# cbrl/BNN-PYNQ

Measured on AMD Instinct MI355X. Metric: images/sec (whole node) CNV-W1A1 CIFAR-10-shape batch, higher is better.
Workload: dtype u1; 1 GPU; cnvW1A1, 131072 synthetic 32x32x3 uint8 images per GPU per step, inputs resident in HBM, params cifar10/cnvW1A1; parallelism=dp1 (batch shards, no data-path collective)

## Files before the change

### bnn-pynq_amd/csrc/kernels.hip

```cpp
#include <hip/hip_runtime.h>
#include <hip/hip_ext.h>
#include <stdint.h>

#include <cstdlib>
#include <cstring>
#include <type_traits>

#define BNN_HD __host__ __device__
#include "act_faults.h"
#include "input_faults.h"
#include "kernels.h"
#include "mem_faults.h"
#include "mem_org.h"
#include "packed_params.h"
static_assert(bnn::kL0TileOffset == (int)bnn::kL0MfmaTileOffset && bnn::kL0BigBytes == (int)bnn::kL0MfmaBigBytes,
              "k_conv0_tile's operand offsets must be the ones packed_params.cpp writes the layer-0 table by");

namespace bnn {
namespace {

typedef const uint32_t __attribute__((address_space(4))) *kptr32;
typedef const uint64_t __attribute__((address_space(4))) *kptr64;

constexpr int kBlock = 256;
constexpr int kLfcFusedMaxA2 = 2048;

struct BlockMap { int cg, item; bool valid; };
__device__ __forceinline__ BlockMap map_block(int groups, int n_items) {
  const int bid = blockIdx.x, xcd = bid & 7, slot = bid >> 3;
  const int sg = slot / groups;
  BlockMap m;
  m.cg = slot - sg * groups;
  m.item = (sg * 8 + xcd) * kBlock + threadIdx.x;
  m.valid = m.item < n_items;
  return m;
}

struct MultiArgs {
  const MultiSeg *segs;
  unsigned stride_dw;
  int ipi;
  int res_images;
};
__device__ __forceinline__ MultiSeg multi_seg(const MultiArgs &ma) {
  kptr32 p = (kptr32)(uintptr_t)(ma.segs + blockIdx.y);
  return MultiSeg{(int)p[0], (int)p[1], (int)p[2], (int)p[3]};
}
template <typename T>
__device__ __forceinline__ int multi_prologue(const MultiArgs &ma, const uint32_t *__restrict__ &rows, T *__restrict__ &out, int &n_items, int out_per_item) {
  const MultiSeg sg = multi_seg(ma);
  rows += (size_t)sg.run * ma.stride_dw;
  n_items = sg.len * ma.ipi;
  if (ma.res_images > 0) out += ((size_t)sg.run * ma.res_images + sg.image - sg.slot) * out_per_item;
  return sg.slot * ma.ipi;
}

__device__ __forceinline__ int pc64(uint64_t x) { return __builtin_popcountll(x); }

__device__ __forceinline__ void mark_done(unsigned *done, unsigned seq, int lane) {
  if (!done) return;
  __threadfence_system();
  if (lane == 0) *reinterpret_cast<volatile unsigned *>(done) = seq;
}

template <bool OUT2, int NPB = 32>
__device__ __forceinline__ void store_bits(uint32_t *__restrict__ out, size_t pix, int groups, int g,
                                           uint32_t b0, uint32_t b1) {
  constexpr int PER64 = 64 / NPB;
  if constexpr (!OUT2) {
    if constexpr (NPB == 32) out[pix * groups + g] = b0;
    else reinterpret_cast<uint8_t *>(out)[pix * groups + g] = (uint8_t)b0;
  } else {
    const size_t w64 = pix * (groups / PER64) + g / PER64;
    const int sub = g % PER64;
    if constexpr (NPB == 32) {
      out[(w64 * 2 + 0) * 2 + sub] = b0;
      out[(w64 * 2 + 1) * 2 + sub] = b1;
    } else {
      uint8_t *o8 = reinterpret_cast<uint8_t *>(out);
      o8[(w64 * 2 + 0) * 8 + sub] = (uint8_t)b0;
      o8[(w64 * 2 + 1) * 8 + sub] = (uint8_t)b1;
    }
  }
}

template <int ARITH>
__device__ __forceinline__ void mac(int &m, int &z, uint64_t as, uint64_t az, kptr64 w) {
  if constexpr (ARITH == AR_XNOR) {
    m += pc64(w[0] ^ as);
  } else if constexpr (ARITH == AR_TB) {
    m += pc64(az & (as ^ w[0]));
  } else {
    const uint64_t zz = az & w[1];
    z += pc64(zz);
    m += pc64(zz & (as ^ w[0]));
  }
}

template <int ARITH>
constexpr int planes_in() { return ARITH == AR_XNOR ? 1 : 2; }
template <int ARITH>
constexpr int wplanes() { return ARITH == AR_TT ? 2 : 1; }
template <int ARITH, int KW>
constexpr int row_dw() { return ARITH == AR_TT ? 4 + 6 * KW : 2 + 2 * KW * wplanes<ARITH>(); }
__device__ __forceinline__ int two_extra(uint32_t two, uint32_t as, uint32_t az) {
  const uint32_t x = two & az;
  return 2 * __builtin_popcount(x & as) - __builtin_popcount(x);
}
__device__ __forceinline__ int two_extra64(uint64_t two, uint64_t as, uint64_t az) {
  const uint64_t x = two & az;
  return 2 * __builtin_popcountll(x & as) - __builtin_popcountll(x);
}

template <int ARITH>
__device__ __forceinline__ int finish(int m, int z, int nzt) {
  if constexpr (ARITH == AR_XNOR) return m;
  else if constexpr (ARITH == AR_TB) return nzt - 2 * m;
  else return z - 2 * m;
}

__device__ __forceinline__ uint32_t quantise4(uint32_t p) {
  const uint32_t t = p ^ 0x80808080u;
  const uint32_t s = (t & 0x7F7F7F7Fu) + 0x01010101u;
  const uint32_t inc = p & ~s & 0x80808080u;
  return t + (inc >> 7);
}

__device__ __forceinline__ uint32_t shift_in_sign(uint32_t bits, int v) {
  asm("" : "+v"(v));
  return __builtin_amdgcn_alignbit(bits, (uint32_t)v, 31);
}

__device__ __forceinline__ void gather_taps(const uint8_t *__restrict__ imgs, int item, uint32_t (&a)[7]) {
  const int img = item / 900, p = item - img * 900;
  const int oy = p / 30, ox = p - oy * 30;
  const uint32_t *__restrict__ im32 = reinterpret_cast<const uint32_t *>(imgs + (size_t)img * 3072);
  const uint32_t *__restrict__ row0 = im32 + oy * 8 + (ox >> 2);
  const int last = 767 - (oy * 8 + (ox >> 2));
  const int sh = ox & 3;
  uint32_t g[9];
#pragma unroll
  for (int c = 0; c < 3; c++)
#pragma unroll
    for (int r = 0; r < 3; r++) {
      const int off = c * 256 + r * 8;
      const uint32_t d0 = row0[off];
      const uint32_t d1 = (c == 2 && r == 2) ? row0[off + 1 <= last ? off + 1 : last] : row0[off + 1];
      g[c * 3 + r] = __builtin_amdgcn_alignbyte(d1, d0, sh);
    }
#pragma unroll
  for (int h = 0; h < 2; h++) {
    a[3 * h + 0] = __builtin_amdgcn_perm(g[4 * h + 1], g[4 * h + 0], 0x04020100u);
    a[3 * h + 1] = __builtin_amdgcn_perm(g[4 * h + 2], g[4 * h + 1], 0x05040201u);
    a[3 * h + 2] = __builtin_amdgcn_perm(g[4 * h + 3], g[4 * h + 2], 0x06050402u);
  }
  a[6] = g[8];
#pragma unroll
  for (int j = 0; j < 7; j++) a[j] = quantise4(a[j]);
}

template <bool OUT2, bool MULTI = false>
__global__ __launch_bounds__(kBlock) void k_conv0(const uint8_t *__restrict__ imgs, uint32_t *__restrict__ out,
                                                   const uint32_t *__restrict__ rows, int n_items, int groups, int gpb, MultiArgs ma = {}) {
  if constexpr (MULTI) {
    const MultiSeg sg = multi_seg(ma);
    rows += (size_t)sg.run * ma.stride_dw;
    n_items = sg.len * 900;
    imgs += (size_t)sg.image * 3072;
    out += (size_t)sg.slot * 900 * (OUT2 ? 4 : 2);
  }
  const BlockMap bm = map_block(groups / gpb, n_items);
  if (!bm.valid) return;
  const int item = bm.item;
  uint32_t a[7];
  gather_taps(imgs, item, a);
  for (int cg = bm.cg * gpb, cg_end = cg + gpb; cg < cg_end; cg++) {
    kptr32 w = (kptr32)(uintptr_t)(rows + (size_t)cg * 32 * 12);
    uint32_t b0 = 0, b1 = 0;
    for (int c = 31; c >= 0; c -= 2) {
      kptr32 rA = w + c * 12, rB = rA - 12;
      int accA = ~(int)rA[0], accB = ~(int)rB[0];
  #pragma unroll
      for (int k = 0; k < 7; k++) {
        accA = __builtin_amdgcn_sdot4((int)a[k], (int)rA[2 + k], accA, false);
        asm("" : "+v"(accA));
        accB = __builtin_amdgcn_sdot4((int)a[k], (int)rB[2 + k], accB, false);
        asm("" : "+v"(accB));
      }
      if constexpr (!OUT2) {
        b0 = shift_in_sign(b0, accA);
        b0 = shift_in_sign(b0, accB);
      } else {
        const int dA = accA + ((int)rA[0] - (int)rA[1]), dB = accB + ((int)rB[0] - (int)rB[1]);
        b0 = shift_in_sign(b0, accA & dA);
        b1 = shift_in_sign(b1, accA ^ dA);
        b0 = shift_in_sign(b0, accB & dB);
        b1 = shift_in_sign(b1, accB ^ dB);
      }
    }
    if constexpr (!OUT2) b0 = ~b0;
    else b1 = ~b1;
    store_bits<OUT2>(out, (size_t)item, 2, cg, b0, b1);
  }
}

typedef int v4i __attribute__((ext_vector_type(4)));
typedef int v16i __attribute__((ext_vector_type(16)));

__device__ __forceinline__ uint32_t sign_nibbles(const int (&v)[16], int h) {
  uint32_t x = 0;
#pragma unroll
  for (int g = 3; g >= 0; g--) {
#pragma unroll
    for (int q = 3; q >= 0; q--) x = shift_in_sign(x, v[4 * g + q]);
    if (g) x <<= 4;
  }
  return x << (4 * h);
}
__device__ __forceinline__ uint32_t or_halves(uint32_t x) {
  const auto sw = __builtin_amdgcn_permlane32_swap(x, x, false, false);
  return sw[0] | sw[1];
}

template <bool OUT2>
__global__ __launch_bounds__(kBlock, 2) void k_conv0_mfma(const uint8_t *__restrict__ imgs, uint32_t *__restrict__ out,
                                                        const uint8_t *__restrict__ l0tab, int n_items) {
  const int lane = threadIdx.x & 63, r = lane & 31, h = lane >> 5;
  const int pix = blockIdx.x * kBlock + threadIdx.x;
  if (pix - lane >= n_items) return;
  uint32_t t[7];
  gather_taps(imgs, pix < n_items ? pix : n_items - 1, t);
  uint32_t lo[4] = {t[0], t[1], t[2], t[3]};
  uint32_t hi[4] = {t[4], t[5], (t[6] & 0x00FFFFFFu) | 0x01000000u, 0x00000040u};
  v4i bp[2];
#pragma unroll
  for (int k = 0; k < 4; k++) {
    const auto sw = __builtin_amdgcn_permlane32_swap(lo[k], hi[k], false, false);
    bp[0][k] = (int)sw[0];
    bp[1][k] = (int)sw[1];
  }
  const v4i *__restrict__ atab = reinterpret_cast<const v4i *>(l0tab);
  uint32_t w0[2] = {0, 0}, w1[2] = {0, 0};
  const v16i zero = {0, 0, 0, 0, 0, 0, 0, 0, 0, 0, 0, 0, 0, 0, 0, 0};
#pragma unroll
  for (int ct = 0; ct < 2; ct++) {
    const v4i a = atab[(32 * ct + r) * 2 + h];
    v4i a2 = a;
    if constexpr (OUT2) a2 = atab[(64 + 32 * ct + r) * 2 + h];
#pragma unroll
    for (int pt = 0; pt < 2; pt++) {
      const v16i acc = __builtin_amdgcn_mfma_i32_32x32x32_i8(a, bp[pt], zero, 0, 0, 0);
      int v[16];
#pragma unroll
      for (int i = 0; i < 16; i++) v[i] = acc[i];
      uint32_t y0, y1 = 0;
      if constexpr (!OUT2) {
        y0 = ~or_halves(sign_nibbles(v, h));
      } else {
        const v16i acc2 = __builtin_amdgcn_mfma_i32_32x32x32_i8(a2, bp[pt], zero, 0, 0, 0);
        int u[16];
#pragma unroll
        for (int i = 0; i < 16; i++) u[i] = acc2[i];
        const uint32_t n0 = sign_nibbles(v, h), n1 = sign_nibbles(u, h);
        y0 = or_halves(n0 & n1);
        y1 = ~or_halves(n0 ^ n1);
      }
      const uint32_t mine = (pt == h) ? 0xFFFFFFFFu : 0u;
      w0[ct] |= y0 & mine;
      w1[ct] |= y1 & mine;
    }
  }
  if (pix < n_items) {
    if constexpr (!OUT2) {
      *reinterpret_cast<uint2 *>(out + (size_t)pix * 2) = make_uint2(w0[0], w0[1]);
    } else {
      *reinterpret_cast<uint4 *>(out + (size_t)pix * 4) = make_uint4(w0[0], w0[1], w1[0], w1[1]);
    }
  }
}

constexpr int kL0Imgs = 8;
constexpr int kL0Plane = 1024 + 64, kL0Image = 3 * kL0Plane;

__device__ __forceinline__ uint32_t sign_bits16(const v16i &acc) {
  uint32_t x = 0;
#pragma unroll
  for (int i = 15; i >= 0; i--) x = shift_in_sign(x, acc[i]);
  return x;
}
__device__ __forceinline__ uint32_t merge_halves(uint32_t a, uint32_t b) {
  const auto sw = __builtin_amdgcn_permlane32_swap(a, b, false, false);
  return sw[0] | sw[1];
}
template <int OFF>
__device__ __forceinline__ uint32_t lds_run(const uint32_t *aligned, uint32_t shift) {
  return __builtin_amdgcn_alignbyte(aligned[OFF / 4 + 1], aligned[OFF / 4], shift);
}

template <bool OUT2, bool MULTI = false>
__global__ __launch_bounds__(kBlock, 2) void k_conv0_tile(const uint8_t *__restrict__ imgs, uint32_t *__restrict__ out,
                                                        const uint8_t *__restrict__ l0tab, int n_images, MultiArgs ma = {}) {
  __shared__ uint4 q4[kL0Imgs * kL0Image / 16];
  const int tid = threadIdx.x, lane = tid & 63, r = lane & 31, h = lane >> 5;
  const int wave = __builtin_amdgcn_readfirstlane(tid >> 6);
  const int img0 = blockIdx.x * kL0Imgs;
  if constexpr (MULTI) {
    const MultiSeg sg = multi_seg(ma);
    if (img0 >= sg.len) return;
    l0tab += (size_t)sg.run * ma.stride_dw * 4;
    n_images = sg.len;
    imgs += (size_t)sg.image * 3072;
    out += (size_t)sg.slot * 900 * (OUT2 ? 4 : 2);
  }
  const int cnt = __builtin_amdgcn_readfirstlane(min(kL0Imgs, n_images - img0));
  const uint4 *__restrict__ src = reinterpret_cast<const uint4 *>(imgs + (size_t)img0 * 3072);
  for (int i = tid; i < cnt * 192; i += kBlock) {
    uint4 v = src[i];
    v.x = quantise4(v.x); v.y = quantise4(v.y); v.z = quantise4(v.z); v.w = quantise4(v.w);
    const int g = i / 192, j = i - g * 192;
    q4[(g * kL0Image + (j >> 6) * kL0Plane + (j & 63) * 16) >> 4] = v;
  }
  const uint8_t *__restrict__ tab = l0tab + kL0TileOffset;
  v4i abig[2];
  long asm0[2], asm1[2];
#pragma unroll
  for (int ct = 0; ct < 2; ct++) {
    abig[ct] = *reinterpret_cast<const v4i *>(tab + ((ct * 32 + r) * 2 + h) * 16);
    asm0[ct] = *reinterpret_cast<const long *>(tab + kL0BigBytes + (((0 * 2 + ct) * 32 + r) * 2 + h) * 8);
    asm1[ct] = OUT2 ? *reinterpret_cast<const long *>(tab + kL0BigBytes + (((1 * 2 + ct) * 32 + r) * 2 + h) * 8) : 0;
  }
  __syncthreads();
  const uint8_t *qb = reinterpret_cast<const uint8_t *>(q4);
  const v16i zero = {0, 0, 0, 0, 0, 0, 0, 0, 0, 0, 0, 0, 0, 0, 0, 0};
  const uint32_t lane_byte = (uint32_t)(r + h * kL0Plane);
  const bool live = r < 30;
  for (int T = wave; T < cnt * 30; T += kBlock / 64) {
    const int gi = T / 30, oy = T - gi * 30;
    const size_t pix = (size_t)(img0 + gi) * 900 + (size_t)(oy * 30) + r;
    const uint32_t byte = (uint32_t)(gi * kL0Image + 32 * oy) + lane_byte;
    const uint32_t *al = reinterpret_cast<const uint32_t *>(qb + (byte & ~3u));
    const uint32_t *al2 = reinterpret_cast<const uint32_t *>(qb + ((byte & ~3u) - h * (kL0Plane - 64)));
    v4i bb;
    bb[0] = (int)lds_run<0>(al, byte);
    bb[1] = (int)lds_run<32>(al, byte);
    bb[2] = (int)lds_run<64>(al, byte);
    bb[3] = (int)lds_run<2 * kL0Plane>(al2, byte);
    const uint32_t mid = lds_run<2 * kL0Plane + 32>(al2, byte);
    const long bs = (long)(uint64_t)(h ? 0x00004001u : mid);
    uint32_t x[2], y[2];
    v16i big[2], d0[2], d1[2];
#pragma unroll
    for (int ct = 0; ct < 2; ct++) big[ct] = __builtin_amdgcn_mfma_i32_32x32x32_i8(abig[ct], bb, zero, 0, 0, 0);
#pragma unroll
    for (int ct = 0; ct < 2; ct++) {
      d0[ct] = __builtin_amdgcn_mfma_i32_32x32x16_i8(asm0[ct], bs, big[ct], 0, 0, 0);
      if constexpr (OUT2) d1[ct] = __builtin_amdgcn_mfma_i32_32x32x16_i8(asm1[ct], bs, big[ct], 0, 0, 0);
    }
#pragma unroll
    for (int ct = 0; ct < 2; ct++) {
      if constexpr (!OUT2) {
        x[ct] = sign_bits16(d0[ct]) << (16 * h);
      } else {
        const uint32_t n0 = sign_bits16(d0[ct]), n1 = sign_bits16(d1[ct]);
        x[ct] = (n0 & n1) << (16 * h);
        y[ct] = (n0 ^ n1) << (16 * h);
      }
    }
    if constexpr (!OUT2) {
      const uint32_t w = ~merge_halves(x[0], x[1]);
      if (live) out[pix * 2 + h] = w;
    } else {
      const uint32_t sg = merge_halves(x[0], x[1]), nz = ~merge_halves(y[0], y[1]);
      if (live) {
        out[pix * 4 + h] = sg;
        out[pix * 4 + 2 + h] = nz;
      }
    }
  }
}

__global__ __launch_bounds__(kBlock) void k_l1_literal(const uint64_t *__restrict__ in, uint64_t *__restrict__ out,
                                                        const uint32_t *__restrict__ rows, int n_items) {
  __shared__ uint64_t w[64][9];
  __shared__ int thr[64];
  for (int i = threadIdx.x; i < 64 * 20; i += kBlock) {
    const int n = i / 20, j = i - n * 20;
    const uint32_t v = rows[i];
    if (j == 0) thr[n] = (int)v;
    else if (j >= 2) reinterpret_cast<uint32_t *>(&w[n][0])[j - 2] = v;
  }
  __syncthreads();
  const int item = blockIdx.x * kBlock + threadIdx.x;
  const int it = item < n_items ? item : n_items - 1;
  const int quad = it >> 2, sub = it & 3, img = quad / 196, q = quad - img * 196, qy = q / 14, qx = q - qy * 14;
  const int oy = 2 * qy + (sub >> 1), ox = 2 * qx + (sub & 1);
  const uint64_t *__restrict__ base = in + (size_t)img * 900 + (size_t)oy * 30 + ox;
  uint64_t a[9];
#pragma unroll
  for (int ky = 0; ky < 3; ky++)
#pragma unroll
    for (int kx = 0; kx < 3; kx++) a[ky * 3 + kx] = base[ky * 30 + kx];
  uint64_t bits = 0;
  for (int n = 0; n < 64; n++) {
    int m = 0;
#pragma unroll
    for (int j = 0; j < 9; j++) m += __popcll(w[n][j] ^ a[j]);
    bits |= (uint64_t)(m < thr[n]) << n;
  }
  bits |= __shfl_xor(bits, 1, 64);
  bits |= __shfl_xor(bits, 2, 64);
  if (sub == 0 && item < n_items) out[quad] = bits;
}

typedef int v8i __attribute__((ext_vector_type(8)));
typedef float v16f __attribute__((ext_vector_type(16)));
constexpr int kL1Pix = 912;

__device__ __forceinline__ uint32_t fp4_pm1(uint32_t byte) {
  uint32_t t = ~byte & 0xFFu;
  t = (t | (t << 12)) & 0x000F000Fu;
  t = (t | (t << 6)) & 0x03030303u;
  t = (t | (t << 3)) & 0x11111111u;
  return (t << 3) + 0x22222222u;
}

__global__ __launch_bounds__(256, 2) void k_l1_mfma(const uint32_t *__restrict__ in, uint32_t *__restrict__ out,
                                                     const uint8_t *__restrict__ tab, int n_images) {
  __shared__ uint4 plane[2][2][kL1Pix];
  __shared__ uint32_t lut[256];
  const int tid = threadIdx.x, lane = tid & 63, wave = tid >> 6, c = lane & 31, h = lane >> 5;
  lut[tid] = fp4_pm1((uint32_t)tid);
  const uint4 *__restrict__ wt = reinterpret_cast<const uint4 *>(tab);
  v8i wreg[9][2];
#pragma unroll
  for (int tap = 0; tap < 9; tap++)
#pragma unroll
    for (int mt = 0; mt < 2; mt++) {
      const uint4 v = wt[(tap * 2 + mt) * 64 + lane];
      wreg[tap][mt] = v8i{(int)v.x, (int)v.y, (int)v.z, (int)v.w, 0, 0, 0, 0};
    }
  __shared__ v16f seed_lds[2][2];
  if (tid < 64) reinterpret_cast<float *>(seed_lds)[tid] = reinterpret_cast<const float *>(tab + kL1MfmaWeights)[tid];
  const int cc = c < 28 ? c : 27;
  uint32_t pre[15];
  auto fetch = [&](int pair) {
    const int img0 = pair * 2, lim = min(2, n_images - img0) * 1800;
#pragma unroll
    for (int j = 0; j < 15; j++) {
      const int d = tid + 256 * j;
      pre[j] = d < lim ? in[(size_t)img0 * 1800 + d] : 0u;
    }
  };
  if (blockIdx.x * 2 < n_images) fetch(blockIdx.x);
  for (int pair = blockIdx.x; pair * 2 < n_images; pair += gridDim.x) {
    const int img0 = pair * 2, nimg = min(2, n_images - img0);
    __syncthreads();
#pragma unroll
    for (int j = 0; j < 15; j++) {
      const int d = tid + 256 * j;
      if (d < nimg * 1800) {
        const int i = d >= 1800, e = d - i * 1800, pix = e >> 1, hh = e & 1;
        const uint32_t bits = pre[j];
        plane[i][hh][pix] = make_uint4(lut[bits & 255], lut[(bits >> 8) & 255], lut[(bits >> 16) & 255], lut[bits >> 24]);
      }
    }
    if ((pair + gridDim.x) * 2 < n_images) fetch(pair + gridDim.x);
    __syncthreads();
    for (int rp = wave; rp < nimg * 14; rp += 4) {
      const int i = rp / 14, r = rp - i * 14;
      const uint4 *__restrict__ P = &plane[i][h][0];
      v16f acc[2][2] = {{seed_lds[0][h], seed_lds[0][h]}, {seed_lds[1][h], seed_lds[1][h]}};
#pragma unroll
      for (int kx = 0; kx < 3; kx++) {
        v8i b[4];
#pragma unroll
        for (int y = 0; y < 4; y++) {
          const uint4 v = P[(2 * r + y) * 30 + cc + kx];
          b[y] = v8i{(int)v.x, (int)v.y, (int)v.z, (int)v.w, 0, 0, 0, 0};
        }
#pragma unroll
        for (int ky = 0; ky < 3; ky++)
#pragma unroll
          for (int mt = 0; mt < 2; mt++)
#pragma unroll
            for (int pt = 0; pt < 2; pt++)
              acc[mt][pt] = __builtin_amdgcn_mfma_scale_f32_32x32x64_f8f6f4(wreg[ky * 3 + kx][mt], b[ky + pt], acc[mt][pt], 4, 4, 0,
                                                                              0x7F7F7F7F, 0, 0x7F7F7F7F);
      }
      uint32_t word[2];
#pragma unroll
      for (int mt = 0; mt < 2; mt++) {
        int v[16];
#pragma unroll
        for (int k = 0; k < 16; k++) v[k] = __float_as_int(fmaxf(acc[mt][0][k], acc[mt][1][k]));
        const uint32_t nf = or_halves(sign_nibbles(v, h));
        const uint32_t pooled = nf & (uint32_t)__builtin_amdgcn_mov_dpp((int)nf, 0xB1, 0xF, 0xF, true);
        word[mt] = ~pooled;
      }
      if (h == 0 && c < 28 && !(c & 1))
        *reinterpret_cast<uint2 *>(out + ((size_t)(img0 + i) * 196 + r * 14 + (c >> 1)) * 2) = make_uint2(word[0], word[1]);
    }
  }
}

constexpr int conv_mfma_row_stride(int win) {
  int ws = win;
  while ((2 * ws - (win - 2)) % 16) ws++;
  return ws;
}
constexpr int conv_mfma_img_stride(int win, int cd) {
  const int ws = conv_mfma_row_stride(win);
  int s = cd * win * ws;
  while ((s - 2 * ((win - 2) / 2 - 1) * ws - (win - 2)) % 16) s++;
  return s;
}

template <int WIN, int CD, int NT, bool POOL, int G>
__global__ __launch_bounds__(256, 2) void k_conv_mfma(const uint32_t *__restrict__ in, uint32_t *__restrict__ out,
                                                       const uint8_t *__restrict__ tab, int n_images) {
  constexpr int WOUT = WIN - 2, RP = WOUT / 2, IPI = RP * WOUT, KH = CD / 2, KS = 9 * KH, NS = 3 * KH, STREAMS = 4 / NT;
  constexpr int PIX = WIN * WIN, DWI = PIX * CD, NPF = (G * DWI + 255) / 256;
  constexpr int WS = conv_mfma_row_stride(WIN), PIXS = WIN * WS, IMGS = conv_mfma_img_stride(WIN, CD);
  static_assert(WOUT % 2 == 0 && IPI % 2 == 0 && (NT == 2 || NT == 4), "tile geometry");
  __shared__ uint4 plane[G * IMGS];
  __shared__ uint32_t lut[256];
  const int tid = threadIdx.x, lane = tid & 63, wave = __builtin_amdgcn_readfirstlane(tid >> 6), mt = wave % NT, c = lane & 31, h = lane >> 5;
  lut[tid] = fp4_pm1((uint32_t)tid);
  const uint4 *__restrict__ wt = reinterpret_cast<const uint4 *>(tab);
  v8i wreg[KS];
#pragma unroll
  for (int ks = 0; ks < KS; ks++) {
    const uint4 v = wt[(ks * NT + mt) * 64 + lane];
    wreg[ks] = v8i{(int)v.x, (int)v.y, (int)v.z, (int)v.w, 0, 0, 0, 0};
  }
  const v16f seed = reinterpret_cast<const v16f *>(tab + (size_t)KS * NT * 64 * 16)[mt * 2 + h];
  const int ngroups = (n_images + G - 1) / G;
  uint32_t pre[NPF];
  auto fetch = [&](int grp) {
    const int img0 = grp * G, lim = min(G, n_images - img0) * DWI;
#pragma unroll
    for (int j = 0; j < NPF; j++) {
      const int d = tid + 256 * j;
      pre[j] = d < lim ? in[(size_t)img0 * DWI + d] : 0u;
    }
  };
  auto slot = [&](int d) {
    const int i = d / DWI, e = d - i * DWI, pix = e / CD, q = e % CD;
    return i * IMGS + q * PIXS + (WS == WIN ? pix : pix / WIN * WS + pix % WIN);
  };
  constexpr int STEP = 32 * STREAMS, DR = STEP / WOUT, DX = STEP % WOUT, PS_LAST = (G - 1) * IMGS + 2 * (RP - 1) * WS + WOUT - 1;
  constexpr bool RAGGED = (G * IPI) % 32 != 0;
  static_assert(DX % 2 == 0 && DR + 1 <= RP, "a lane's column keeps its parity; one row-pair wrap and one image wrap per step");
  const int item0 = (wave / NT) * 32 + c, i0 = item0 / IPI, rem0 = item0 - i0 * IPI, rp0 = rem0 / WOUT, x0 = rem0 - rp0 * WOUT;
  const int ps0 = i0 * IMGS + 2 * rp0 * WS + x0;
  const uint32_t ob0 = (uint32_t)((i0 * (WOUT * WOUT) + (2 * rp0 + h) * WOUT + x0) * NT + mt) * 4;
  if (blockIdx.x < ngroups) fetch(blockIdx.x);
  for (int grp = blockIdx.x; grp < ngroups; grp += gridDim.x) {
    const int img0 = grp * G, nimg = min(G, n_images - img0), nitems = nimg * IPI;
    uint32_t *__restrict__ gout = out + (size_t)img0 * (POOL ? RP * RP : WOUT * WOUT) * NT;
    __syncthreads();
#pragma unroll
    for (int j = 0; j < NPF; j++) {
      const int d = tid + 256 * j;
      if (d < nimg * DWI) {
        const uint32_t bits = pre[j];
        plane[slot(d)] = make_uint4(lut[bits & 255], lut[(bits >> 8) & 255], lut[(bits >> 16) & 255], lut[bits >> 24]);
      }
    }
    if (grp + (int)gridDim.x < ngroups) fetch(grp + gridDim.x);
    __syncthreads();
    int x = x0, rp = rp0, ps = ps0;
    [[maybe_unused]] uint32_t ob = ob0;
    for (int t0 = (wave / NT) * 32; t0 < nitems; t0 += STEP) {
      v16f acc[2] = {seed, seed};
      const uint4 *__restrict__ P = &plane[(RAGGED ? min(ps, PS_LAST) : ps) + h * PIXS];
      auto read = [&](v8i &b, int s, int y) {
        const uint4 v = P[(s / 3) * 2 * PIXS + y * WS + s % 3];
        b = v8i{(int)v.x, (int)v.y, (int)v.z, (int)v.w, 0, 0, 0, 0};
      };
      auto mfma = [&](const v8i (&b)[4], int s, int k) {
        acc[k & 1] = __builtin_amdgcn_mfma_scale_f32_32x32x64_f8f6f4(wreg[((k >> 1) * 3 + s % 3) * KH + s / 3], b[(k >> 1) + (k & 1)], acc[k & 1], 4,
                                                                    4, 0, 0x7F7F7F7F, 0, 0x7F7F7F7F);
      };
      v8i b[2][4];
#pragma unroll
      for (int y = 0; y < 4; y++) read(b[0][y], 0, y);
#pragma unroll
      for (int s = 0; s < NS; s++)
#pragma unroll
        for (int k = 0; k < 6; k++) {
          __builtin_amdgcn_sched_barrier(0);
          mfma(b[s & 1], s, k);
          if (s + 1 < NS && k < 4) read(b[(s + 1) & 1][k], s + 1, k);
        }
      __builtin_amdgcn_sched_barrier(0);
      const bool valid = t0 + c < nitems;
      if constexpr (POOL) {
        int v[16];
#pragma unroll
        for (int k = 0; k < 16; k++) v[k] = __float_as_int(acc[0][k]) & __float_as_int(acc[1][k]);
        const uint32_t nf = or_halves(sign_nibbles(v, h));
        const uint32_t pooled = nf & (uint32_t)__builtin_amdgcn_mov_dpp((int)nf, 0xB1, 0xF, 0xF, true);
        if (valid && h == 0 && !(c & 1)) gout[(size_t)(t0 >> 1) * NT + (c >> 1) * NT + mt] = ~pooled;
      } else {
        uint32_t nf[2];
#pragma unroll
        for (int dy = 0; dy < 2; dy++) {
          int v[16];
#pragma unroll
          for (int k = 0; k < 16; k++) v[k] = __float_as_int(acc[dy][k]);
          nf[dy] = sign_nibbles(v, h);
        }
        const auto sw = __builtin_amdgcn_permlane32_swap(nf[0], nf[1], false, false);
        if (valid) *reinterpret_cast<uint32_t *>(reinterpret_cast<char *>(gout) + ob) = ~(sw[0] | sw[1]);
      }
      x += DX, rp += DR, ps += 2 * DR * WS + DX;
      if constexpr (!POOL) ob += (2 * DR * WOUT + DX) * NT * 4;
      if (x >= WOUT) {
        x -= WOUT, rp += 1, ps += 2 * WS - WOUT;
        if constexpr (!POOL) ob += WOUT * NT * 4;
      }
      if (rp >= RP) rp -= RP, ps += IMGS - 2 * RP * WS;
    }
  }
}

__global__ __launch_bounds__(256) void k_conv_mfma_table(const uint32_t *__restrict__ rows, int row_dw, int ksteps, int tiles,
                                                          int mw, uint8_t *__restrict__ dst) {
  const int idx = blockIdx.x * 256 + threadIdx.x, nw = ksteps * tiles * 64;
  if (idx < nw) {
    const int ks = idx / (tiles * 64), mt = (idx / 64) % tiles, lane = idx & 63, n = 32 * mt + (lane & 31), h = lane >> 5;
    const uint32_t bits = rows[(size_t)n * row_dw + 2 + 2 * ks + h];
    reinterpret_cast<uint4 *>(dst)[idx] = make_uint4(fp4_pm1(bits & 255), fp4_pm1((bits >> 8) & 255), fp4_pm1((bits >> 16) & 255),
                                                     fp4_pm1(bits >> 24));
  } else if (idx < nw + tiles * 32) {
    const int j = idx - nw, mt = j >> 5, h = (j >> 4) & 1, reg = j & 15;
    const int n = 32 * mt + (reg & 3) + 8 * (reg >> 2) + 4 * h;
    long long t = (int)rows[(size_t)n * row_dw];
    t = t < -1 ? -1 : (t > mw + 2 ? mw + 2 : t);
    reinterpret_cast<float *>(dst + (size_t)nw * 16)[j] = (float)(-(mw - 2 * t) - 1);
  }
}

__device__ __forceinline__ uint32_t nibble_spread(uint32_t byte) {
  uint32_t t = byte & 0xFFu;
  t = (t | (t << 12)) & 0x000F000Fu;
  t = (t | (t << 6)) & 0x03030303u;
  return (t | (t << 3)) & 0x11111111u;
}
__device__ __forceinline__ uint4 fp4_planes(const uint32_t *lutz, const uint32_t *luts, uint32_t sg, uint32_t nz) {
  const uint32_t m = sg & nz;
  return make_uint4(lutz[nz & 255] | luts[m & 255], lutz[(nz >> 8) & 255] | luts[(m >> 8) & 255],
                    lutz[(nz >> 16) & 255] | luts[(m >> 16) & 255], lutz[nz >> 24] | luts[m >> 24]);
}
__device__ __forceinline__ void not_fired(const v16f &acc, const v16f &dt, int h, uint32_t &n0, uint32_t &n1) {
  int v[16], u[16];
#pragma unroll
  for (int k = 0; k < 16; k++) {
    v[k] = __float_as_int(acc[k]);
    u[k] = __float_as_int(acc[k] - dt[k]);
  }
  n0 = or_halves(sign_nibbles(v, h));
  n1 = or_halves(sign_nibbles(u, h));
}

template <int WIN, int CD, int NT, bool POOL, int G>
__global__ __launch_bounds__(256, 2) void k_conv_mfma_a2(const uint4 *__restrict__ in, uint32_t *__restrict__ out,
                                                          const uint8_t *__restrict__ tab, int n_images) {
  constexpr int WOUT = WIN - 2, RP = WOUT / 2, IPI = RP * WOUT, KH = CD / 2, KS = 9 * KH, STREAMS = 4 / NT;
  constexpr int PIX = WIN * WIN, QWI = PIX * KH, NPF = (G * QWI + 255) / 256;
  static_assert(WOUT % 2 == 0 && IPI % 2 == 0 && (NT == 2 || NT == 4), "tile geometry");
  __shared__ uint4 plane[G][CD][PIX];
  __shared__ uint32_t lutz[256], luts[256];
  const int tid = threadIdx.x, lane = tid & 63, wave = tid >> 6, mt = wave % NT, c = lane & 31, h = lane >> 5;
  lutz[tid] = nibble_spread((uint32_t)tid) << 1;
  luts[tid] = nibble_spread((uint32_t)tid) << 3;
  const uint4 *__restrict__ wt = reinterpret_cast<const uint4 *>(tab);
  v8i wreg[KS];
#pragma unroll
  for (int ks = 0; ks < KS; ks++) {
    const uint4 v = wt[(ks * NT + mt) * 64 + lane];
    wreg[ks] = v8i{(int)v.x, (int)v.y, (int)v.z, (int)v.w, 0, 0, 0, 0};
  }
  const v16f *__restrict__ cst = reinterpret_cast<const v16f *>(tab + (size_t)KS * NT * 64 * 16);
  const v16f seed = cst[mt * 2 + h], dt = cst[NT * 2 + mt * 2 + h];
  const int ngroups = (n_images + G - 1) / G;
  uint4 pre[NPF];
  auto fetch = [&](int grp) {
    const int img0 = grp * G, lim = min(G, n_images - img0) * QWI;
#pragma unroll
    for (int j = 0; j < NPF; j++) {
      const int d = tid + 256 * j;
      pre[j] = d < lim ? in[(size_t)img0 * QWI + d] : make_uint4(0u, 0u, 0u, 0u);
    }
  };
  if (blockIdx.x < ngroups) fetch(blockIdx.x);
  for (int grp = blockIdx.x; grp < ngroups; grp += gridDim.x) {
    const int img0 = grp * G, nimg = min(G, n_images - img0), nitems = nimg * IPI;
    __syncthreads();
#pragma unroll
    for (int j = 0; j < NPF; j++) {
      const int d = tid + 256 * j;
      if (d < nimg * QWI) {
        const int i = d / QWI, e = d - i * QWI, pix = e / KH, cw = e % KH;
        const uint4 v = pre[j];
        plane[i][2 * cw][pix] = fp4_planes(lutz, luts, v.x, v.z);
        plane[i][2 * cw + 1][pix] = fp4_planes(lutz, luts, v.y, v.w);
      }
    }
    if (grp + (int)gridDim.x < ngroups) fetch(grp + gridDim.x);
    __syncthreads();
    for (int t0 = (wave / NT) * 32; t0 < nitems; t0 += 32 * STREAMS) {
      const int item = min(t0 + c, nitems - 1);
      const int i = item / IPI, rem = item - i * IPI, rp = rem / WOUT, x = rem - rp * WOUT;
      v16f acc[2] = {seed, seed};
#pragma unroll
      for (int kh = 0; kh < KH; kh++) {
        const uint4 *__restrict__ P = &plane[i][kh * 2 + h][2 * rp * WIN + x];
#pragma unroll
        for (int kx = 0; kx < 3; kx++) {
          v8i b[4];
#pragma unroll
          for (int y = 0; y < 4; y++) {
            const uint4 v = P[y * WIN + kx];
            b[y] = v8i{(int)v.x, (int)v.y, (int)v.z, (int)v.w, 0, 0, 0, 0};
          }
#pragma unroll
          for (int ky = 0; ky < 3; ky++)
#pragma unroll
            for (int dy = 0; dy < 2; dy++)
              acc[dy] = __builtin_amdgcn_mfma_scale_f32_32x32x64_f8f6f4(wreg[(ky * 3 + kx) * KH + kh], b[ky + dy], acc[dy], 4, 4, 0,
                                                                         0x7F7F7F7F, 0, 0x7F7F7F7F);
        }
      }
      const bool valid = t0 + c < nitems;
      const size_t img = (size_t)(img0 + i);
      if constexpr (POOL) {
        v16f top;
#pragma unroll
        for (int k = 0; k < 16; k++) top[k] = fmaxf(acc[0][k], acc[1][k]);
        uint32_t n0, n1;
        not_fired(top, dt, h, n0, n1);
        n0 &= (uint32_t)__builtin_amdgcn_mov_dpp((int)n0, 0xB1, 0xF, 0xF, true);
        n1 &= (uint32_t)__builtin_amdgcn_mov_dpp((int)n1, 0xB1, 0xF, 0xF, true);
        const size_t w64 = (img * (RP * RP) + rp * RP + (x >> 1)) * (NT / 2) + mt / 2;
        if (valid && !(x & 1)) out[(w64 * 2 + h) * 2 + (mt & 1)] = h ? ~(n0 ^ n1) : (n0 & n1);
      } else {
        uint32_t n0[2], n1[2];
#pragma unroll
        for (int dy = 0; dy < 2; dy++) not_fired(acc[dy], dt, h, n0[dy], n1[dy]);
        const uint32_t m0 = h ? n0[1] : n0[0], m1 = h ? n1[1] : n1[0];
        const size_t w64 = (img * (WOUT * WOUT) + (2 * rp + h) * WOUT + x) * (NT / 2) + mt / 2;
        if (valid) {
          out[(w64 * 2 + 0) * 2 + (mt & 1)] = m0 & m1;
          out[(w64 * 2 + 1) * 2 + (mt & 1)] = ~(m0 ^ m1);
        }
      }
    }
  }
}

template <bool TT>
__global__ __launch_bounds__(256) void k_conv_mfma_a2_table(const uint32_t *__restrict__ rows, int ksteps, int tiles,
                                                             uint8_t *__restrict__ dst) {
  const int idx = blockIdx.x * 256 + threadIdx.x, nw = ksteps * tiles * 64, row_dw = TT ? 4 + 6 * ksteps : 2 + 2 * ksteps;
  if (idx < nw) {
    const int ks = idx / (tiles * 64), mt = (idx / 64) % tiles, lane = idx & 63, n = 32 * mt + (lane & 31), h = lane >> 5;
    const uint32_t *__restrict__ row = rows + (size_t)n * row_dw;
    uint32_t b1, b2 = 0, b3;
    if constexpr (TT) {
      const uint32_t sg = row[2 + 4 * ks + h], two = row[2 + 4 * ksteps + 2 * ks + h], nz = row[2 + 4 * ks + 2 + h] | two;
      b1 = nz & ~two;
      b2 = two;
      b3 = (sg & nz) | two;
    } else {
      b1 = 0xFFFFFFFFu;
      b3 = row[2 + 2 * ks + h];
    }
    uint32_t v[4];
#pragma unroll
    for (int k = 0; k < 4; k++)
      v[k] = (nibble_spread(b1 >> (8 * k)) << 1) | (nibble_spread(b2 >> (8 * k)) << 2) | (nibble_spread(b3 >> (8 * k)) << 3);
    reinterpret_cast<uint4 *>(dst)[idx] = make_uint4(v[0], v[1], v[2], v[3]);
  } else if (idx < nw + tiles * 64) {
    const int j = idx - nw, second = j >= tiles * 32, jj = second ? j - tiles * 32 : j, mt = jj >> 5, h = (jj >> 4) & 1, reg = jj & 15;
    const int n = 32 * mt + (reg & 3) + 8 * (reg >> 2) + 4 * h;
    const int lim = 2 * 64 * ksteps;
    int t0 = (int)rows[(size_t)n * row_dw], t1 = (int)rows[(size_t)n * row_dw + 1];
    t0 = t0 < -lim - 1 ? -lim - 1 : (t0 > lim ? lim : t0);
    t1 = t1 < -lim - 1 ? -lim - 1 : (t1 > lim ? lim : t1);
    reinterpret_cast<float *>(dst + (size_t)nw * 16)[j] = second ? (float)(t1 - t0) : -(float)t0 - 0.5f;
  }
}

template <bool A2, int KS, int NT, bool CONV, int WAVES, int G>
__global__ __launch_bounds__(64 * WAVES, 8 / WAVES) void k_tail_mfma(const std::conditional_t<A2, uint4, uint32_t> *__restrict__ in,
                                                                      uint32_t *__restrict__ out, const uint8_t *__restrict__ tab,
                                                                      int n_images) {
  using U = std::conditional_t<A2, uint4, uint32_t>;
  constexpr int T = 64 * WAVES, TPW = NT / WAVES, IPI = CONV ? 9 : 1, W64 = CONV ? 25 * 2 : KS, UPI = A2 ? W64 : 2 * W64;
  constexpr int GP = G + 1, NPL = CONV ? G * 4 * 25 : 2 * KS * GP, NPF = (G * UPI + T - 1) / T, NC = (A2 ? 2 : 1) * NT * 2;
  static_assert(NT % WAVES == 0 && (!CONV || KS == 18) && (G * IPI) % 32 == 0, "tile geometry");
  __shared__ uint4 plane[NPL];
  __shared__ uint32_t lut[A2 ? 512 : 256];
  __shared__ v16f cst[NC];
  const int tid = threadIdx.x, lane = tid & 63, wave = tid >> 6, mt0 = wave * TPW, c = lane & 31, h = lane >> 5;
  for (int k = tid; k < 256; k += T) {
    if constexpr (A2) {
      lut[k] = nibble_spread((uint32_t)k) << 1;
      lut[256 + k] = nibble_spread((uint32_t)k) << 3;
    } else {
      lut[k] = fp4_pm1((uint32_t)k);
    }
  }
  for (int k = tid; k < NC * 16; k += T) reinterpret_cast<float *>(cst)[k] = reinterpret_cast<const float *>(tab + (size_t)KS * NT * 64 * 16)[k];
  const uint4 *__restrict__ wt = reinterpret_cast<const uint4 *>(tab);
  v8i wreg[TPW][KS];
#pragma unroll
  for (int j = 0; j < TPW; j++)
#pragma unroll
    for (int ks = 0; ks < KS; ks++) {
      const uint4 v = wt[(ks * NT + mt0 + j) * 64 + lane];
      wreg[j][ks] = v8i{(int)v.x, (int)v.y, (int)v.z, (int)v.w, 0, 0, 0, 0};
    }
  const int ngroups = (n_images + G - 1) / G;
  U pre[NPF];
  auto fetch = [&](int grp) {
    const int img0 = grp * G, lim = min(G, n_images - img0) * UPI;
#pragma unroll
    for (int j = 0; j < NPF; j++) {
      const int d = tid + T * j;
      pre[j] = d < lim ? in[(size_t)img0 * UPI + d] : U{};
    }
  };
  if (blockIdx.x < ngroups) fetch(blockIdx.x);
  for (int grp = blockIdx.x; grp < ngroups; grp += gridDim.x) {
    const int img0 = grp * G, nimg = min(G, n_images - img0), nitems = nimg * IPI;
    __syncthreads();
#pragma unroll
    for (int j = 0; j < NPF; j++) {
      const int d = tid + T * j;
      if (d < nimg * UPI) {
        const int i = d / UPI, e = d - i * UPI;
        if constexpr (A2) {
          const uint4 v = pre[j];
          const int p0 = CONV ? (i * 4 + 2 * (e & 1)) * 25 + (e >> 1) : 2 * e * GP + i, step = CONV ? 25 : GP;
          plane[p0] = fp4_planes(lut, lut + 256, v.x, v.z);
          plane[p0 + step] = fp4_planes(lut, lut + 256, v.y, v.w);
        } else {
          const uint32_t bits = pre[j];
          const int p0 = CONV ? (i * 4 + (e & 3)) * 25 + (e >> 2) : e * GP + i;
          plane[p0] = make_uint4(lut[bits & 255], lut[(bits >> 8) & 255], lut[(bits >> 16) & 255], lut[bits >> 24]);
        }
      }
    }
    if (grp + (int)gridDim.x < ngroups) fetch(grp + gridDim.x);
    __syncthreads();
#pragma unroll 1
    for (int t0 = 0; t0 < nitems; t0 += 32) {
      const int item = min(t0 + c, nitems - 1);
      int base;
      if constexpr (CONV) {
        const int i = item / 9, p = item - i * 9, oy = p / 3, ox = p - oy * 3;
        base = (i * 4 + h) * 25 + oy * 5 + ox;
      } else {
        base = h * GP + item;
      }
      v16f acc[TPW];
#pragma unroll
      for (int j = 0; j < TPW; j++) acc[j] = cst[(mt0 + j) * 2 + h];
#pragma unroll
      for (int ks = 0; ks < KS; ks++) {
        const int off = CONV ? (ks & 1) * 2 * 25 + ((ks >> 1) / 3) * 5 + (ks >> 1) % 3 : ks * 2 * GP;
        const uint4 v = plane[base + off];
        const v8i b = v8i{(int)v.x, (int)v.y, (int)v.z, (int)v.w, 0, 0, 0, 0};
#pragma unroll
        for (int j = 0; j < TPW; j++)
          acc[j] = __builtin_amdgcn_mfma_scale_f32_32x32x64_f8f6f4(wreg[j][ks], b, acc[j], 4, 4, 0, 0x7F7F7F7F, 0, 0x7F7F7F7F);
      }
      const bool valid = t0 + c < nitems;
      const size_t gitem = (size_t)img0 * IPI + item;
#pragma unroll
      for (int j = 0; j < TPW; j++) {
        const int mt = mt0 + j;
        if constexpr (A2) {
          uint32_t n0, n1;
          not_fired(acc[j], cst[NT * 2 + mt * 2 + h], h, n0, n1);
          const size_t w64 = gitem * (NT / 2) + mt / 2;
          if (valid) out[(w64 * 2 + h) * 2 + (mt & 1)] = h ? ~(n0 ^ n1) : (n0 & n1);
        } else {
          int v[16];
#pragma unroll
          for (int k = 0; k < 16; k++) v[k] = __float_as_int(acc[j][k]);
          const uint32_t nf = or_halves(sign_nibbles(v, h));
          if (valid && h == (j & 1)) out[gitem * NT + mt] = ~nf;
        }
      }
    }
  }
}

__device__ __forceinline__ uint32_t chain_temp() {
  uint32_t t;
  asm("" : "=v"(t));
  return t;
}
#ifdef BNN_VGPR_COUNTER
#define SCALAR_COUNTER(c) do { } while (0)
#else
#define SCALAR_COUNTER(c) asm volatile("" : "+s"(c))
#endif
__device__ __forceinline__ void xpop(int &acc, uint32_t w, uint32_t a, uint32_t &t) {
  asm("v_xor_b32 %0, %2, %3\n\tv_bcnt_u32_b32 %1, %0, %1" : "+v"(t), "+v"(acc) : "s"(w), "v"(a));
}
__device__ __forceinline__ void xpop4(int &m0, int &m1, int &m2, int &m3, uint32_t w, uint32_t a0, uint32_t a1,
                                      uint32_t a2, uint32_t a3, uint32_t &t) {
  xpop(m0, w, a0, t); xpop(m1, w, a1, t); xpop(m2, w, a2, t); xpop(m3, w, a3, t);
}
__device__ __forceinline__ int xpop_seed(uint32_t w, uint32_t a, int seed, uint32_t &t) {
  int acc;
  asm("v_xor_b32 %0, %2, %3\n\tv_bcnt_u32_b32 %1, %0, %4" : "+v"(t), "=v"(acc) : "s"(w), "v"(a), "s"(seed));
  return acc;
}
template <int NPB>
__device__ __forceinline__ void store_group(uint32_t *__restrict__ out, size_t index, uint32_t bits) {
  if constexpr (NPB == 32) out[index] = bits;
  else reinterpret_cast<uint8_t *>(out)[index] = (uint8_t)bits;
}

template <int CW, int ID, bool POOL, int NPB = 32, bool MULTI = false>
__global__ __launch_bounds__(kBlock) void k_quad_x(const uint64_t *__restrict__ in, uint32_t *__restrict__ out,
                                                    const uint32_t *__restrict__ rows, int n_items, int groups, int gpb, MultiArgs ma = {}) {
  constexpr int OD = ID - 2, QD = OD / 2, NQ = QD * QD, KW = 9 * CW, ROW_DW = 2 + 2 * KW;
  int item0 = 0;
  if constexpr (MULTI) item0 = multi_prologue(ma, rows, out, n_items, 0);
  const BlockMap bm = map_block(groups / gpb, n_items);
  if (!bm.valid) return;
  const int item = bm.item + item0;
  const int img = item / NQ, q = item - img * NQ;
  const int qy = q / QD, qx = q - qy * QD;
  const uint64_t *__restrict__ base = in + ((size_t)img * ID * ID + (size_t)(2 * qy) * ID + 2 * qx) * CW;
  uint32_t wl[4][4][CW], wh[4][4][CW];
#pragma unroll
  for (int y = 0; y < 4; y++)
#pragma unroll
    for (int x = 0; x < 4; x++)
#pragma unroll
      for (int k = 0; k < CW; k++) {
        const uint64_t v = base[(y * ID + x) * CW + k];
        wl[y][x][k] = (uint32_t)v;
        wh[y][x][k] = (uint32_t)(v >> 32);
      }
  uint32_t t = chain_temp();
  for (int cg = bm.cg * gpb, cg_end = cg + gpb; cg < cg_end; cg++) {
    kptr32 w = (kptr32)(uintptr_t)(rows + (size_t)cg * NPB * ROW_DW);
    uint32_t b[4] = {0, 0, 0, 0};
    for (int c = NPB - 1; c >= 0; c--) {
      kptr32 r = w + c * ROW_DW;
      SCALAR_COUNTER(c);
      const int nt = -(int)r[0];
      int m[2][2];
  #pragma unroll
      for (int j = 0; j < KW; j++) {
        const int ky = j / (3 * CW), kx = (j / CW) % 3, k = j % CW;
        const uint32_t w0 = r[2 + 2 * j], w1 = r[3 + 2 * j];
        if (j == 0) {
  #pragma unroll
          for (int i = 0; i < 4; i++) m[i >> 1][i & 1] = xpop_seed(w0, wl[ky + (i >> 1)][kx + (i & 1)][k], nt, t);
        } else {
          xpop4(m[0][0], m[0][1], m[1][0], m[1][1], w0, wl[ky][kx][k], wl[ky][kx + 1][k], wl[ky + 1][kx][k], wl[ky + 1][kx + 1][k], t);
        }
        xpop4(m[0][0], m[0][1], m[1][0], m[1][1], w1, wh[ky][kx][k], wh[ky][kx + 1][k], wh[ky + 1][kx][k], wh[ky + 1][kx + 1][k], t);
      }
      if constexpr (POOL) {
        b[0] = shift_in_sign(b[0], min(min(m[0][0], m[0][1]), min(m[1][0], m[1][1])));
      } else {
  #pragma unroll
        for (int i = 0; i < 4; i++) b[i] = shift_in_sign(b[i], m[i >> 1][i & 1]);
      }
    }
    if constexpr (POOL) {
      store_group<NPB>(out, (size_t)item * groups + cg, b[0]);
    } else {
  #pragma unroll
      for (int i = 0; i < 4; i++) {
        const size_t pix = (size_t)img * OD * OD + (size_t)(2 * qy + (i >> 1)) * OD + 2 * qx + (i & 1);
        store_group<NPB>(out, pix * groups + cg, b[i]);
      }
    }
  }
}

template <int KW, int NPB>
__device__ __forceinline__ uint32_t vec_x_group(kptr32 w, const uint32_t (&al)[KW], const uint32_t (&ah)[KW], uint32_t &t) {
  constexpr int ROW_DW = 2 + 2 * KW;
  uint32_t b = 0;
  for (int c = NPB - 1; c >= 0; c -= 2) {
    kptr32 r1 = w + c * ROW_DW, r0 = r1 - ROW_DW;
    int m1 = xpop_seed(r1[2], al[0], -(int)r1[0], t), m0 = xpop_seed(r0[2], al[0], -(int)r0[0], t);
    xpop(m1, r1[3], ah[0], t);
    xpop(m0, r0[3], ah[0], t);
#pragma unroll
    for (int k = 1; k < KW; k++) {
      xpop(m1, r1[2 + 2 * k], al[k], t);
      xpop(m0, r0[2 + 2 * k], al[k], t);
      xpop(m1, r1[3 + 2 * k], ah[k], t);
      xpop(m0, r0[3 + 2 * k], ah[k], t);
    }
    b = shift_in_sign(b, m1);
    b = shift_in_sign(b, m0);
  }
  return b;
}

template <int KW, bool SINGLE, int CW, int ID, int NPB = 32, bool POOL = false, bool MULTI = false>
__global__ __launch_bounds__(kBlock) void k_vec_x(const uint64_t *__restrict__ in, uint32_t *__restrict__ out,
                                                   const uint32_t *__restrict__ rows, int n_items, int groups, int gpb, MultiArgs ma = {}) {
  constexpr int ROW_DW = 2 + 2 * KW;
  static_assert(!POOL || SINGLE, "pooling needs the window form");
  static_assert(!MULTI || NPB == 32, "multi-run launches use the 32-neuron form");
  int item0 = 0;
  if constexpr (MULTI) item0 = multi_prologue(ma, rows, out, n_items, groups);
  const BlockMap bm = map_block(groups / gpb, n_items);
  if (!bm.valid) return;
  const int item = bm.item + item0;
  uint32_t al[KW], ah[KW];
  if constexpr (SINGLE) {
    constexpr int OD = ID - 2;
    static_assert(KW == 9 * CW, "window size");
    int img, oy, ox;
    if constexpr (POOL) {
      constexpr int QD = OD / 2, NQ = QD * QD;
      const int quad = item >> 2, sub = item & 3;
      img = quad / NQ;
      const int q = quad - img * NQ, qy = q / QD, qx = q - qy * QD;
      oy = 2 * qy + (sub >> 1);
      ox = 2 * qx + (sub & 1);
    } else {
      img = item / (OD * OD);
      const int p = item - img * (OD * OD);
      oy = p / OD;
      ox = p - oy * OD;
    }
    const uint64_t *__restrict__ base = in + ((size_t)img * ID * ID + (size_t)oy * ID + ox) * CW;
#pragma unroll
    for (int ky = 0; ky < 3; ky++)
#pragma unroll
      for (int kx = 0; kx < 3; kx++)
#pragma unroll
        for (int k = 0; k < CW; k++) {
          const uint64_t v = base[(ky * ID + kx) * CW + k];
          al[(ky * 3 + kx) * CW + k] = (uint32_t)v;
          ah[(ky * 3 + kx) * CW + k] = (uint32_t)(v >> 32);
        }
  } else {
    const uint64_t *__restrict__ base = in + (size_t)item * KW;
#pragma unroll
    for (int k = 0; k < KW; k++) {
      const uint64_t v = base[k];
      al[k] = (uint32_t)v;
      ah[k] = (uint32_t)(v >> 32);
    }
  }
  uint32_t t = chain_temp();
  for (int cg = bm.cg * gpb, cg_end = cg + gpb; cg < cg_end; cg++) {
    kptr32 w = (kptr32)(uintptr_t)(rows + (size_t)cg * NPB * ROW_DW);
    uint32_t b = 0;
    for (int c = NPB - 1; c >= 0; c -= 2) {
      kptr32 r1 = w + c * ROW_DW, r0 = r1 - ROW_DW;
      int m1 = xpop_seed(r1[2], al[0], -(int)r1[0], t), m0 = xpop_seed(r0[2], al[0], -(int)r0[0], t);
      xpop(m1, r1[3], ah[0], t);
      xpop(m0, r0[3], ah[0], t);
  #pragma unroll
      for (int k = 1; k < KW; k++) {
        xpop(m1, r1[2 + 2 * k], al[k], t);
        xpop(m0, r0[2 + 2 * k], al[k], t);
        xpop(m1, r1[3 + 2 * k], ah[k], t);
        xpop(m0, r0[3 + 2 * k], ah[k], t);
      }
      b = shift_in_sign(b, m1);
      b = shift_in_sign(b, m0);
    }
    if constexpr (POOL) {
      b |= __shfl_xor(b, 1, 64);
      b |= __shfl_xor(b, 2, 64);
      if ((item & 3) == 0) store_group<NPB>(out, (size_t)(item >> 2) * groups + cg, b);
    } else {
      store_group<NPB>(out, (size_t)item * groups + cg, b);
    }
  }
}


#define BNN_BITOP_AND_XOR "0x28"

template <int ARITH, bool FIRST = false>
__device__ __forceinline__ void mac32(int &m, int &z, uint32_t as, uint32_t az, kptr32 wq, int half, uint32_t &t, int seed = 0) {
  if constexpr (ARITH == AR_XNOR) {
    if constexpr (FIRST) asm("v_xor_b32 %0, %2, %3\n\tv_bcnt_u32_b32 %1, %0, %4" : "+v"(t), "=v"(m) : "s"(wq[half]), "v"(as), "s"(seed));
    else asm("v_xor_b32 %0, %2, %3\n\tv_bcnt_u32_b32 %1, %0, %1" : "+v"(t), "+v"(m) : "s"(wq[half]), "v"(as));
  } else if constexpr (ARITH == AR_TB) {
    if constexpr (FIRST)
      asm("v_bitop3_b32 %0, %2, %3, %4 bitop3:" BNN_BITOP_AND_XOR "\n\tv_bcnt_u32_b32 %1, %0, 0"
          : "+v"(t), "=v"(m)
          : "s"(wq[half]), "v"(as), "v"(az));
    else
      asm("v_bitop3_b32 %0, %2, %3, %4 bitop3:" BNN_BITOP_AND_XOR "\n\tv_bcnt_u32_b32 %1, %0, %1"
          : "+v"(t), "+v"(m)
          : "s"(wq[half]), "v"(as), "v"(az));
  } else {
    if constexpr (FIRST) {
      asm("v_and_b32 %0, %2, %3\n\tv_bcnt_u32_b32 %1, %0, 0" : "+v"(t), "=v"(z) : "s"(wq[2 + half]), "v"(az));
      asm("v_bitop3_b32 %0, %2, %3, %0 bitop3:" BNN_BITOP_AND_XOR "\n\tv_bcnt_u32_b32 %1, %0, 0" : "+v"(t), "=v"(m) : "s"(wq[half]), "v"(as));
    } else {
      asm("v_and_b32 %0, %2, %3\n\tv_bcnt_u32_b32 %1, %0, %1" : "+v"(t), "+v"(z) : "s"(wq[2 + half]), "v"(az));
      asm("v_bitop3_b32 %0, %2, %3, %0 bitop3:" BNN_BITOP_AND_XOR "\n\tv_bcnt_u32_b32 %1, %0, %1" : "+v"(t), "+v"(m) : "s"(wq[half]), "v"(as));
    }
  }
}

template <int ARITH>
__device__ __forceinline__ int d_of(int m, int zz) {
  int d;
  asm("v_mad_i32_i24 %0, %1, -2, %2" : "=v"(d) : "v"(m), "v"(zz));
  return d;
}

template <bool OUT2>
__device__ __forceinline__ void decide(uint32_t &b0, uint32_t &b1, int g0, int dt) {
  b0 = shift_in_sign(b0, g0);
  if constexpr (OUT2) b1 = shift_in_sign(b1, g0 + dt);
}
template <bool OUT2>
__device__ __forceinline__ void finish_bits(uint32_t &b0, uint32_t &b1) {
  if constexpr (OUT2) {
    const uint32_t f0 = b0, f1 = b1;
    b0 = ~(f0 | f1);
    b1 = ~(f0 ^ f1);
  }
}

template <int ARITH, int CW, int ID, bool POOL, bool OUT2, int NPB = 32, bool TWO = false, bool MULTI = false>
__global__ __launch_bounds__(kBlock) void k_quad(const uint64_t *__restrict__ in, uint32_t *__restrict__ out,
                                                  const uint32_t *__restrict__ rows, int n_items, int groups, int gpb, MultiArgs ma = {}) {
  constexpr int OD = ID - 2, QD = OD / 2, NQ = QD * QD, PL = planes_in<ARITH>(), WPL = wplanes<ARITH>();
  constexpr int KW = 9 * CW, ROW_DW = row_dw<ARITH, KW>(), ZW = (PL == 2) ? CW : 1;
  int item0 = 0;
  if constexpr (MULTI) item0 = multi_prologue(ma, rows, out, n_items, 0);
  const BlockMap bm = map_block(groups / gpb, n_items);
  if (!bm.valid) return;
  const int item = bm.item + item0;
  const int img = item / NQ, q = item - img * NQ;
  const int qy = q / QD, qx = q - qy * QD;
  const uint64_t *__restrict__ base = in + ((size_t)img * ID * ID + (size_t)(2 * qy) * ID + 2 * qx) * CW * PL;
  uint32_t ws[4][4][CW][2], wz[4][4][ZW][2];
#pragma unroll
  for (int y = 0; y < 4; y++)
#pragma unroll
    for (int x = 0; x < 4; x++)
#pragma unroll
      for (int k = 0; k < CW; k++) {
// ... 2224 lines not shown
```

Measured before the change: 39.12 million images/s.

## Software-pipeline LDS loads in conv0 tile kernel and simplify staging/stores

Reworks the layer-0 MFMA conv kernel: image staging now loads one plane per wave with direct indexing, LDS operand words for the next tile are prefetched during the current tile's MFMAs, the bs operand is built with an inline-asm alignbyte under a forced exec mask, and output addressing uses precomputed per-lane byte offsets with a 16-bit merge instead of shifting. The aim is to hide LDS latency and cut integer address arithmetic in the hot loop, at the cost of more live registers and fragile inline asm that overrides exec.

```diff
diff --git a/bnn-pynq_amd/csrc/kernels.hip b/bnn-pynq_amd/csrc/kernels.hip
--- a/bnn-pynq_amd/csrc/kernels.hip
+++ b/bnn-pynq_amd/csrc/kernels.hip
@@ -288,13 +288,9 @@
   for (int i = 15; i >= 0; i--) x = shift_in_sign(x, acc[i]);
   return x;
 }
-__device__ __forceinline__ uint32_t merge_halves(uint32_t a, uint32_t b) {
+__device__ __forceinline__ uint32_t merge_halves16(uint32_t a, uint32_t b) {
   const auto sw = __builtin_amdgcn_permlane32_swap(a, b, false, false);
-  return sw[0] | sw[1];
-}
-template <int OFF>
-__device__ __forceinline__ uint32_t lds_run(const uint32_t *aligned, uint32_t shift) {
-  return __builtin_amdgcn_alignbyte(aligned[OFF / 4 + 1], aligned[OFF / 4], shift);
+  return sw[0] | (sw[1] << 16);
 }
 
 template <bool OUT2, bool MULTI = false>
@@ -313,12 +309,13 @@
     out += (size_t)sg.slot * 900 * (OUT2 ? 4 : 2);
   }
   const int cnt = __builtin_amdgcn_readfirstlane(min(kL0Imgs, n_images - img0));
-  const uint4 *__restrict__ src = reinterpret_cast<const uint4 *>(imgs + (size_t)img0 * 3072);
-  for (int i = tid; i < cnt * 192; i += kBlock) {
-    uint4 v = src[i];
+  static_assert(kL0Image == 3 * kL0Plane && kL0Plane % 16 == 0, "the planes of a block follow each other at one stride");
+  const uint8_t *__restrict__ src = imgs + (size_t)img0 * 3072;
+#pragma clang loop unroll(disable) interleave(disable) vectorize(disable)
+  for (int p = wave; p < cnt * 3; p += kBlock / 64) {
+    uint4 v = *reinterpret_cast<const uint4 *>(src + (size_t)p * 1024 + (uint32_t)lane * 16);
     v.x = quantise4(v.x); v.y = quantise4(v.y); v.z = quantise4(v.z); v.w = quantise4(v.w);
-    const int g = i / 192, j = i - g * 192;
-    q4[(g * kL0Image + (j >> 6) * kL0Plane + (j & 63) * 16) >> 4] = v;
+    q4[p * (kL0Plane / 16) + lane] = v;
   }
   const uint8_t *__restrict__ tab = l0tab + kL0TileOffset;
   v4i abig[2];
@@ -332,21 +329,40 @@
   __syncthreads();
   const uint8_t *qb = reinterpret_cast<const uint8_t *>(q4);
   const v16i zero = {0, 0, 0, 0, 0, 0, 0, 0, 0, 0, 0, 0, 0, 0, 0, 0};
+  constexpr int W = OUT2 ? 4 : 2;
   const uint32_t lane_byte = (uint32_t)(r + h * kL0Plane);
+  const uint32_t al_lane = lane_byte & ~3u;
+  uint32_t al2_lane = al_lane + 2 * kL0Plane - h * (kL0Plane - 64);
+  uint32_t lane_out = (uint32_t)(r * W + h) * 4;
+  asm("" : "+v"(al2_lane), "+v"(lane_out));
   const bool live = r < 30;
-  for (int T = wave; T < cnt * 30; T += kBlock / 64) {
+  const int tiles = cnt * 30;
+  uint32_t lo[5], hi[5];
+  const auto fetch = [&](int T) {
     const int gi = T / 30, oy = T - gi * 30;
-    const size_t pix = (size_t)(img0 + gi) * 900 + (size_t)(oy * 30) + r;
-    const uint32_t byte = (uint32_t)(gi * kL0Image + 32 * oy) + lane_byte;
-    const uint32_t *al = reinterpret_cast<const uint32_t *>(qb + (byte & ~3u));
-    const uint32_t *al2 = reinterpret_cast<const uint32_t *>(qb + ((byte & ~3u) - h * (kL0Plane - 64)));
+    const uint32_t tile = (uint32_t)(gi * kL0Image + 32 * oy);
+    const uint32_t *al = reinterpret_cast<const uint32_t *>(qb + (al_lane + tile));
+    const uint32_t *al2 = reinterpret_cast<const uint32_t *>(qb + (al2_lane + tile));
+#pragma unroll
+    for (int i = 0; i < 3; i++) lo[i] = al[8 * i], hi[i] = al[8 * i + 1];
+#pragma unroll
+    for (int i = 0; i < 2; i++) lo[3 + i] = al2[8 * i], hi[3 + i] = al2[8 * i + 1];
+  };
+  uint32_t bs_lo = 0x00004001u;
+  fetch(wave);
+  for (int T = wave; T < tiles; T += kBlock / 64) {
+    uint8_t *orow = reinterpret_cast<uint8_t *>(out + ((size_t)img0 * 900 + (size_t)T * 30) * W);
+    asm volatile("" : "+v"(lane_out));
     v4i bb;
-    bb[0] = (int)lds_run<0>(al, byte);
-    bb[1] = (int)lds_run<32>(al, byte);
-    bb[2] = (int)lds_run<64>(al, byte);
-    bb[3] = (int)lds_run<2 * kL0Plane>(al2, byte);
-    const uint32_t mid = lds_run<2 * kL0Plane + 32>(al2, byte);
-    const long bs = (long)(uint64_t)(h ? 0x00004001u : mid);
+#pragma unroll
+    for (int i = 0; i < 4; i++) bb[i] = (int)__builtin_amdgcn_alignbyte(hi[i], lo[i], lane_byte);
+    {
+      uint64_t saved;
+      asm volatile("s_mov_b64 %1, exec\n\ts_mov_b64 exec, 0xffffffff\n\tv_alignbyte_b32 %0, %2, %3, %4\n\ts_mov_b64 exec, %1"
+                   : "+v"(bs_lo), "=&s"(saved)
+                   : "v"(hi[4]), "v"(lo[4]), "v"(lane_byte));
+    }
+    const long bs = (long)(uint64_t)bs_lo;
     uint32_t x[2], y[2];
     v16i big[2], d0[2], d1[2];
 #pragma unroll
@@ -356,24 +372,25 @@
       d0[ct] = __builtin_amdgcn_mfma_i32_32x32x16_i8(asm0[ct], bs, big[ct], 0, 0, 0);
       if constexpr (OUT2) d1[ct] = __builtin_amdgcn_mfma_i32_32x32x16_i8(asm1[ct], bs, big[ct], 0, 0, 0);
     }
+    fetch(min(T + kBlock / 64, tiles - 1));
 #pragma unroll
     for (int ct = 0; ct < 2; ct++) {
       if constexpr (!OUT2) {
-        x[ct] = sign_bits16(d0[ct]) << (16 * h);
+        x[ct] = sign_bits16(d0[ct]);
       } else {
         const uint32_t n0 = sign_bits16(d0[ct]), n1 = sign_bits16(d1[ct]);
-        x[ct] = (n0 & n1) << (16 * h);
-        y[ct] = (n0 ^ n1) << (16 * h);
+        x[ct] = n0 & n1;
+        y[ct] = n0 ^ n1;
       }
     }
     if constexpr (!OUT2) {
-      const uint32_t w = ~merge_halves(x[0], x[1]);
-      if (live) out[pix * 2 + h] = w;
+      const uint32_t w = ~merge_halves16(x[0], x[1]);
+      if (live) *reinterpret_cast<uint32_t *>(orow + lane_out) = w;
     } else {
-      const uint32_t sg = merge_halves(x[0], x[1]), nz = ~merge_halves(y[0], y[1]);
+      const uint32_t sg = merge_halves16(x[0], x[1]), nz = ~merge_halves16(y[0], y[1]);
       if (live) {
-        out[pix * 4 + h] = sg;
-        out[pix * 4 + 2 + h] = nz;
+        *reinterpret_cast<uint32_t *>(orow + lane_out) = sg;
+        *reinterpret_cast<uint32_t *>(orow + lane_out + 8) = nz;
       }
     }
   }
@@ -856,7 +873,7 @@
     }
     if (grp + (int)gridDim.x < ngroups) fetch(grp + gridDim.x);
     __syncthreads();
-#pragma unroll 1
+#pragma clang loop unroll(disable) interleave(disable) vectorize(disable)
     for (int t0 = 0; t0 < nitems; t0 += 32) {
       const int item = min(t0 + c, nitems - 1);
       int base;
```

After: 39.76 million images/s (median of 6 runs). 1.02x the previous value.
